# braingeneers/statdepth

Measured on AMD Instinct MI355X. Metric: curve-pairs/sec (MBD), higher is better.
Workload: dtype f64

## Files before the change

### statdepth_amd/csrc/mbd_rank_bucket32.hip

```cpp
#include <atomic>

#include "sd_common.h"
#include "rank_routes.h"
#include "rank_bucket.h"

namespace sd {

constexpr int R32_PRIO_LDS = 2;
constexpr int R32_PRIO_VALU = 0;
constexpr int R32_MIN_N = 3072;
constexpr int R32_LNB = 14;
constexpr int R32_NT = 512, R32_NW = 8;
constexpr int R32_LCAP = 64;
constexpr int R32_PAD = 12;
constexpr u32 R32_TB = 1024;
constexpr int R32_TSH = 30;
constexpr double R32_CDIV = 1.0 / 448.0;
constexpr double R32_BETA = 2.0;
constexpr u32 R32_SENT = 0x7FFFFFFFu;

template <int E, int LNB>
struct R32Cfg {
    static constexpr int NT = R32_NT, NW = R32_NW, NB = 1 << LNB;
    static constexpr int QW = NB / 2 / NT / 4;
    static_assert(QW >= 1 && NB / 2 == QW * 4 * NT, "whole quads of histogram words per thread");
    static constexpr int SH = 31 - LNB;
    static constexpr u32 C0 = R32_TB << SH, C1 = ((u32)NB - R32_TB) << SH;
    static constexpr u32 NANIMG = ((u32)NB + 2u) << SH;
    static_assert(LNB == 14, "the first tail octave continues the core's slope for 14 336 core buckets");
    static constexpr size_t HDR = 8 * NW * 8 + NW * 4 + 32 + (size_t)R32_LCAP * 8;
    static_assert(HDR % 16 == 0, "the histogram starts on a 16-byte boundary");
    static __host__ __device__ constexpr int al4(int n) { return (n + 3) & ~3; }
    static __host__ __device__ constexpr int pstride(int n) { return (n + 31) & ~31; }
    static __host__ __device__ constexpr int dummy_pos(int n) { return al4(n) + R32_PAD; }
    static __host__ __device__ constexpr size_t lds_bytes(int n) { return HDR + (size_t)(NB / 2 + 4) * 4 + (size_t)(dummy_pos(n) + 4) * 4; }
};

template <int E, int LNB>
__global__ __launch_bounds__(R32_NT, 4) void rank_bucket32_kernel(const double *__restrict__ Y, i64 n64, i64 row0, i64 rows,
                                                                 u32 *__restrict__ partial, unsigned char *__restrict__ rowflag,
                                                                 u32 *__restrict__ gate, u32 epoch, u64 *__restrict__ out_zero) {
    using C = R32Cfg<E, LNB>;
    constexpr int NT = C::NT, NW = C::NW, NB = C::NB, QW = C::QW, SH = C::SH;
    constexpr u32 C0 = C::C0, C1 = C::C1, NANIMG = C::NANIMG;
    extern __shared__ double Sm[];
    const int n = (int)n64;
    double *red = Sm;
    u32 *wtot = reinterpret_cast<u32 *>(red + 8 * NW);
    u32 *misc = wtot + NW;
    u32 *lkey = misc + 8, *lbe = lkey + R32_LCAP;
    u32 *H = reinterpret_cast<u32 *>(reinterpret_cast<char *>(Sm) + C::HDR);
    u32 *S = H + NB / 2 + 4;
    const unsigned short *H16 = reinterpret_cast<const unsigned short *>(H);
    const int t0 = threadIdx.x;
    const double INF = __builtin_huge_val();
    const double QNAN = __builtin_nan("");
    const int DUMMY = C::dummy_pos(n);
    const uint4 *SENT = reinterpret_cast<const uint4 *>(S + C::al4(n));
    const u32 nm1 = (u32)n - 1u;
    const u32 ranksum = (u32)(((u64)n * (u64)(n - 1)) >> 1);
    int t = t0;

    if (blockIdx.x == 0 && t == 0) gate[2] = 0;
    if (out_zero)
        for (i64 c = (i64)blockIdx.x * NT + t; c < n; c += (i64)gridDim.x * NT) out_zero[c] = 0;
    for (int p = n + t; p < DUMMY + 4; p += NT) S[p] = R32_SENT;
    {
        uint4 *Hq = reinterpret_cast<uint4 *>(H);
#pragma unroll
        for (int i = 0; i < QW; ++i) Hq[i * NT + t] = make_uint4(0, 0, 0, 0);
        if (t < 4) H[NB / 2 + t] = 0;
        if (t < 5) misc[t] = 0;
    }

    double x[E];
    auto load_row = [&](i64 r) {
        const double *rp = Y + (row0 + r) * n + t;
#pragma unroll
        for (int e = 0; e < E; ++e) x[e] = (e < E - 2 || t + e * NT < n) ? rp[e * NT] : QNAN;
    };
    u32 acc[E];
#pragma unroll
    for (int e = 0; e < E; ++e) acc[e] = 0;
    double smp;
    auto sample_issue = [&](i64 r) { smp = Y[(row0 + r) * n + (((((u32)t * 397u) & 511u) * (u32)n) >> 9)]; };
    auto row_range = [&](int parity) {
        double mn = INF, mx = -INF;
#pragma unroll
        for (int e = 0; e < E; ++e) {
            mn = rb_mm<false>(mn, x[e]);
            mx = rb_mm<true>(mx, x[e]);
        }
        mn = rb_wave_allreduce<false>(mn);
        mx = rb_wave_allreduce<true>(mx);
        const float sf = (float)smp;
        const float rmn = rb_row_allreduce_f32<false>(sf == sf ? sf : __builtin_huge_valf());
        const float rmx = rb_row_allreduce_f32<true>(sf == sf ? sf : -__builtin_huge_valf());
        auto rl = [](float v, int l) -> float { return __int_as_float(__builtin_amdgcn_readlane(__float_as_int(v), l)); };
        float imn = fmaxf(fmaxf(rl(rmn, 0), rl(rmn, 16)), fmaxf(rl(rmn, 32), rl(rmn, 48)));
        float imx = fminf(fminf(rl(rmx, 0), rl(rmx, 16)), fminf(rl(rmx, 32), rl(rmx, 48)));
        {
            bool eqs = false;
#define R32_NB(k) eqs = eqs || (__int_as_float(__builtin_amdgcn_mov_dpp(__float_as_int(sf), 0x120 + k, 0xF, 0xF, false)) == sf);
            R32_NB(1) R32_NB(2) R32_NB(3) R32_NB(4) R32_NB(5) R32_NB(6) R32_NB(7)
#undef R32_NB
            if (__ballot(eqs) != 0) { imn = __builtin_huge_valf(); imx = -__builtin_huge_valf(); }
        }
        double *rp = red + parity * 4 * NW;
        if ((t & 63) == 63) {
            double *wp = rp + 4 * (t >> 6);
            wp[0] = mn; wp[1] = mx;
            reinterpret_cast<float *>(wp + 2)[0] = imn;
            reinterpret_cast<float *>(wp + 2)[1] = imx;
        }
    };
    int par = 0;
    u32 rowidx = 0, nbad = 0, expect = 0;
    bool handover = false;
    bool stop = false;
    u32 kb[E];
    i64 r = blockIdx.x;
    for (; r < rows; r += gridDim.x) {
        t = t0;
        asm volatile("" : "+v"(t));
        const int lane = t & 63;
        const int wave = __builtin_amdgcn_readfirstlane(t >> 6);
        if (rowidx && t == 0) misc[3] = __hip_atomic_load(gate + 1, __ATOMIC_RELAXED, __HIP_MEMORY_SCOPE_AGENT);
        __builtin_amdgcn_s_setprio(R32_PRIO_LDS);
        sample_issue(r);
        load_row(r);
        row_range(par);
        double *redp = red + par * 4 * NW;
        par ^= 1;
        __syncthreads();
        if (rowidx) {
            const u32 w = misc[3];
            if ((w >> 8) == (epoch & 0xFFFFFFu) && (w & 0xFFu) >= 8u) { stop = true; break; }
        }
        double lo, hi;
        double mscale, moff, mc;
        u64 mcb;
        u32 mc0, mcw;
        bool go, bad;
        {
            const double2 p = reinterpret_cast<const double2 *>(redp)[2 * (lane & (NW - 1))];
            const float2 pb = reinterpret_cast<const float2 *>(redp + 4 * (lane & (NW - 1)) + 2)[0];
            lo = rb_readlane_f64(rb_row_allreduce<false>(p.x), 0);
            hi = rb_readlane_f64(rb_row_allreduce<true>(p.y), 0);
            const double imn = (double)__int_as_float(__builtin_amdgcn_readfirstlane(__float_as_int(rb_row_allreduce_f32<true>(pb.x))));
            const double imx = (double)__int_as_float(__builtin_amdgcn_readfirstlane(__float_as_int(rb_row_allreduce_f32<false>(pb.y))));
            const bool fin = (hi > lo) && (lo > -INF) && (hi < INF) && ((hi - lo) < INF);
            bad = !fin && (hi >= lo);
            const double si = imx - imn;
            u32 c0 = 256u, c1 = 0x7FFFFE00u;
            if (fin && si > 0.0 && si < INF && (hi - lo) > (1.5 * (1.0 + 2.0 * R32_BETA)) * si) {
                const double lo2 = imn - R32_BETA * si, hi2 = imx + R32_BETA * si;
                lo = lo2 > lo ? lo2 : lo;
                hi = hi2 < hi ? hi2 : hi;
                c0 = C0;
                c1 = C1;
            }
            mc0 = c0;
            mcw = c1 - c0;
            const double wc = hi - lo;
            mscale = ((double)mcw - 64.0) / wc;
            moff = __builtin_fma(-lo, mscale, (double)c0);
            mc = wc * R32_CDIV;
            mcb = (u64)__double_as_longlong(mc);
            go = fin && (wc > 0.0) && (mscale < INF) && (mc > 0.0);
            bad = bad || (fin && !go);
        }
        auto convert4 = [&](const double (&xv)[4], u32 (&q)[4], u32 (&bk)[4]) {
            bool anyout = false;
            u32 fr[4];
#pragma unroll
            for (int i = 0; i < 4; ++i) {
                const double u = __builtin_fma(xv[i], mscale, moff);
                u32 qi;
                asm("v_cvt_u32_f64 %0, %1" : "=v"(qi) : "v"(u));
                const double f = __builtin_amdgcn_fract(u) * 16384.0;
                asm("v_cvt_u32_f64 %0, %1" : "=v"(fr[i]) : "v"(f));
                q[i] = qi;
                anyout = anyout || (qi - mc0 >= mcw);
            }
            if (__ballot(anyout) != 0) {
#pragma unroll
                for (int i = 0; i < 4; ++i) {
                    const bool outc = q[i] - mc0 >= mcw, low = q[i] < mc0;
                    double d = low ? lo - xv[i] : xv[i] - hi;
                    d = rb_mm<true>(d, 0.0);
                    const u64 tc = ((u64)__double_as_longlong(d + mc) - mcb) >> R32_TSH;
                    const u32 room = low ? mc0 - 1u : 0x7FFFFEFFu - (mc0 + mcw);
                    const u32 tcc = tc < (u64)room ? (u32)tc : room;
                    u32 qt = low ? (mc0 - 1u) - tcc : (mc0 + mcw) + tcc;
                    qt = (xv[i] == xv[i]) ? qt : NANIMG;
                    q[i] = outc ? qt : q[i];
                    fr[i] = outc ? 0u : fr[i];
                }
            }
#pragma unroll
            for (int i = 0; i < 4; ++i) {
                bk[i] = q[i] >> SH;
                q[i] = ((q[i] << (31 - SH)) & 0x7FFFFFFFu) | fr[i];
            }
        };
        u32 bc[E];
        if (go) {

#pragma unroll
            for (int e0 = 0; e0 < E; e0 += 8) {
                u32 old[8];
#pragma unroll
                for (int h = 0; h < 8; h += 4) {
                    if (e0 + h < E) {
                        double xv[4];
                        u32 q[4], bk[4];
#pragma unroll
                        for (int i = 0; i < 4; ++i) xv[i] = e0 + h + i < E ? x[e0 + h + i] : x[e0 + h];
                        convert4(xv, q, bk);
#pragma unroll
                        for (int i = 0; i < 4; ++i)
                            if (e0 + h + i < E) { kb[e0 + h + i] = q[i]; bc[e0 + h + i] = bk[i]; }
                    }
                }
#pragma unroll
                for (int i = 0; i < 8; ++i) {
                    const int e = e0 + i;
                    if (e < E) {
                        const u32 b = bc[e];
                        old[i] = atomicAdd(&H[b >> 1], 1u << ((b & 1u) * 16u));
                    }
                }
#pragma unroll
                for (int i = 0; i < 8; ++i) {
                    const int e = e0 + i;
                    if (e < E)
                        bc[e] |= ((old[i] >> ((bc[e] & 1u) * 16u)) & 0xFFu) << 16;
                }
#pragma unroll
                for (int i = 0; i < 8; ++i)
                    if (e0 + i < E) asm volatile("" : "+v"(bc[e0 + i]));
            }
            __syncthreads();
            uint4 *Hq = reinterpret_cast<uint4 *>(H) + wave * (64 * QW);
            uint4 hq[QW];
            u32 runq[QW], inclq[QW], offq[QW], ov = 0, wsum = 0;
#pragma unroll
            for (int i = 0; i < QW; ++i) {
                hq[i] = Hq[i * 64 + lane];
                const u32 s4 = hq[i].x + hq[i].y + hq[i].z + hq[i].w;
                ov |= hq[i].x | hq[i].y | hq[i].z | hq[i].w;
                runq[i] = (s4 & 0xFFFFu) + (s4 >> 16);
                inclq[i] = rb_wave_incl_scan(runq[i]);
                offq[i] = wsum;
                wsum += rb_readlane(inclq[i], 63);
            }
            const bool wover = __ballot((ov & 0xFFC0FFC0u) != 0) != 0;
            const bool wtry = __ballot((ov & 0xFFF0FFF0u) != 0) != 0;
            if (lane == 63) wtot[wave] = wsum | (wover ? 0x80000000u : 0u) | (wtry ? 0x40000000u : 0u);
            __syncthreads();
            const u32 wt = wtot[lane & (NW - 1)];
            const bool crowded = __ballot((wt >> 31) != 0) != 0;
            const bool trypure = __ballot((wt & 0x40000000u) != 0) != 0;
            const u32 wscan = rb_row_incl_scan(wt & 0x3FFFFFFFu);
            const u32 woff = wave ? rb_readlane(wscan, wave - 1) : 0u;
#pragma unroll
            for (int i = 0; i < QW; ++i) {
                u32 base = woff + offq[i] + inclq[i] - runq[i];
                uint4 o;
                o.x = base | ((base + (hq[i].x & 0xFFFFu)) << 16);
                base += (hq[i].x & 0xFFFFu) + (hq[i].x >> 16);
                o.y = base | ((base + (hq[i].y & 0xFFFFu)) << 16);
                base += (hq[i].y & 0xFFFFu) + (hq[i].y >> 16);
                o.z = base | ((base + (hq[i].z & 0xFFFFu)) << 16);
                base += (hq[i].z & 0xFFFFu) + (hq[i].z >> 16);
                o.w = base | ((base + (hq[i].w & 0xFFFFu)) << 16);
                base += (hq[i].w & 0xFFFFu) + (hq[i].w >> 16);
                Hq[i * 64 + lane] = o;
                if (i == QW - 1 && t == NT - 1) H[NB / 2] = base;
            }
            __syncthreads();
            const u32 nv = H[NB / 2];
            bool take = nv == (u32)n;
            if (take) {
#pragma unroll
                for (int e = 0; e < E; ++e) {
                    const u32 b = bc[e] & 0xFFFFu, slot = bc[e] >> 16;
                    u32 b1 = b + 1u;
                    asm("" : "+v"(b1));
                    const u32 base = H16[b], end = H16[b1];
                    const bool isk = e < E - 2 || t + e * NT < n;
                    S[isk ? base + slot : (u32)DUMMY] = kb[e];
                    bc[e] = isk ? base | ((end - base) << 14) : (1u << 14);
                }
            }
            __syncthreads();
            bool pure = false;
            if (take && (trypure || crowded)) {
                const u32 tag = rowidx + 1u;
                bool vote = false, same = true;
#pragma unroll
                for (int e = 0; e < E; ++e) {
                    const u32 base = bc[e] & 0x3FFFu, cnt = bc[e] >> 14;
                    if (e < E - 2 || t + e * NT < n) {
                        const u32 first = S[base];
                        same = same && (first == kb[e]);
                        if (cnt >= 16u) vote = vote || (first == kb[e] && S[base + 1] == kb[e]);
                    }
                }
                if (vote) misc[2] = tag;
                if (!same) misc[4] = tag;
                __syncthreads();
                if ((misc[2] == tag && misc[4] != tag) || crowded) {
                    take = false;
                    bool ok = misc[2] == tag && misc[4] != tag;
                    if (ok) {
                        const double *rp = Y + (row0 + r) * n + t;
#pragma unroll
                        for (int pass = 0; pass < 2; ++pass) {
                            bool eq = true;
#pragma unroll
                            for (int e0 = 0; e0 < E; e0 += 4) {
                                int eo = e0 * NT;
                                asm volatile("" : "+v"(eo));
                                const double *rq = rp + eo;
                                u64 w[4];
#pragma unroll
                                for (int i = 0; i < 4; ++i) {
                                    const bool isk = e0 + i < E && (e0 + i < E - 2 || t + (e0 + i) * NT < n);
                                    w[i] = (u64)__double_as_longlong((isk ? rq[i * NT] : 0.0) + 0.0);
                                }
#pragma unroll
                                for (int i = 0; i < 4; ++i) {
                                    if (e0 + i < E && (e0 + i < E - 2 || t + (e0 + i) * NT < n) && (bc[e0 + i] >> 14) >= 2u) {
                                        u32 *sp = S + (bc[e0 + i] & 0x3FFFu);
                                        if (pass == 0) { sp[0] = (u32)(w[i] >> 32); sp[1] = (u32)w[i]; }
                                        else eq = eq && sp[0] == (u32)(w[i] >> 32) && sp[1] == (u32)w[i];
                                    }
                                }
                                __builtin_amdgcn_sched_barrier(0);
                            }
                            if (pass == 1 && !eq) misc[4] = tag;
                            __syncthreads();
                        }
                        ok = misc[4] != tag;
                    }
                    if (ok) {
                        pure = true;
#pragma unroll
                        for (int e = 0; e < E; ++e) {
                            const u32 B = bc[e] & 0x3FFFu, A = (u32)n - B - (bc[e] >> 14);
                            acc[e] += (e < E - 2 || t + e * NT < n) ? (nm1 * (nm1 - 1u) - A * (A - 1u) - B * (B - 1u)) >> 1 : 0u;
                        }
                    }
                }
            }
            __builtin_amdgcn_s_setprio(R32_PRIO_VALU);
            {
                uint4 *Hz = reinterpret_cast<uint4 *>(H) + wave * (64 * QW);
#pragma unroll
                for (int i = 0; i < QW; ++i) Hz[i * 64 + lane] = make_uint4(0, 0, 0, 0);
                if (t < 2) H[NB / 2 + t] = 0;
            }
            if (take) {
                const uint4 *S4 = reinterpret_cast<const uint4 *>(S);
                uint4 y0, y1;
                auto window = [&](int e) {
                    const u32 base = bc[e] & 0x3FFFu, cnt = bc[e] >> 14;
                    const uint4 *p = S4 + (base >> 2);
                    y0 = p[0];
                    y1 = *((cnt + (base & 3u) > 4u) ? p + 1 : SENT);
                };
                u32 sB = 0;
                window(0);
#pragma unroll
                for (int e = 0; e < E; ++e) {
                    const u32 base = bc[e] & 0x3FFFu, cnt = bc[e] >> 14, off = base & 3u;
                    const u32 qe = kb[e];
                    u32 lt = 0;
                    lt = __builtin_amdgcn_alignbit(lt, y1.w - qe, 31);
                    lt = __builtin_amdgcn_alignbit(lt, y1.z - qe, 31);
                    lt = __builtin_amdgcn_alignbit(lt, y1.y - qe, 31);
                    lt = __builtin_amdgcn_alignbit(lt, y1.x - qe, 31);
                    lt = __builtin_amdgcn_alignbit(lt, y0.w - qe, 31);
                    lt = __builtin_amdgcn_alignbit(lt, y0.z - qe, 31);
                    lt = __builtin_amdgcn_alignbit(lt, y0.y - qe, 31);
                    lt = __builtin_amdgcn_alignbit(lt, y0.x - qe, 31);
                    if (e + 1 < E) window(e + 1);
                    u32 less = (u32)__popc(__builtin_amdgcn_ubfe(lt, off, cnt < 8u ? cnt : 8u));
                    if (cnt + off > 8u) {
                        const uint4 *p = S4 + (base >> 2);
#pragma unroll 1
                        for (u32 kk = 8; kk < cnt + off; kk += 4) {
                            const uint4 y = p[kk >> 2];
                            const u32 rest = cnt + off - kk;
                            u32 l4 = 0;
                            l4 = __builtin_amdgcn_alignbit(l4, y.w - qe, 31);
                            l4 = __builtin_amdgcn_alignbit(l4, y.z - qe, 31);
                            l4 = __builtin_amdgcn_alignbit(l4, y.y - qe, 31);
                            l4 = __builtin_amdgcn_alignbit(l4, y.x - qe, 31);
                            less += (u32)__popc(__builtin_amdgcn_ubfe(l4, 0u, rest < 4u ? rest : 4u));
                        }
                    }
                    const u32 B = base + less;
                    kb[e] = B;
                    const bool isk = e < E - 2 || t + e * NT < n;
                    sB += isk ? B : 0u;
                    acc[e] += isk ? __umul24(B, nm1 - B) : 0u;
                    __builtin_amdgcn_sched_barrier(0);
                }
                sB = rb_wave_incl_scan(sB);
                if (lane == 63) atomicAdd(&misc[1], sB);
                __syncthreads();
                {
                    const u32 have_sum = misc[1];
                    expect += ranksum;
                    if (have_sum != expect) {
                        expect = have_sum;
                        const u32 l0 = misc[0];
#pragma unroll
                        for (int e = 0; e < E; ++e)
                            if (e < E - 2 || t + e * NT < n) atomicAdd(&H[kb[e] >> 1], 1u << ((kb[e] & 1u) * 16u));
                        __syncthreads();
#pragma unroll
                        for (int e = 0; e < E; ++e) {
                            if (e < E - 2 || t + e * NT < n) {
                                const u32 B = kb[e], c = H16[B];
                                if (c != 1u) {
                                    acc[e] -= __umul24(B, nm1 - B);
                                    const u32 idx = atomicAdd(&misc[0], 1u);
                                    if (idx < (u32)R32_LCAP) {
                                        lkey[idx] = (rowidx << 14) | (u32)(t + e * NT);
                                        lbe[idx] = B | (c << 16);
                                    }
                                }
                            }
                        }
                        __syncthreads();
                        if (E <= 16 && misc[0] > (u32)R32_LCAP) {
                            const u32 tag = (rowidx + 1u) | 0x40000000u;
                            const double *rp = Y + (row0 + r) * n + t;
#pragma unroll
                            for (int pass = 0; pass < 2; ++pass) {
                                bool eq = true;
#pragma unroll
                                for (int e0 = 0; e0 < E; e0 += 2) {
                                    int eo = e0 * NT;
                                    asm volatile("" : "+v"(eo));
                                    const double *rq = rp + eo;
                                    u64 w[2];
#pragma unroll
                                    for (int i = 0; i < 2; ++i) {
                                        const bool isk = e0 + i < E && (e0 + i < E - 2 || t + (e0 + i) * NT < n);
                                        w[i] = (u64)__double_as_longlong((isk ? rq[i * NT] : 0.0) + 0.0);
                                    }
#pragma unroll
                                    for (int i = 0; i < 2; ++i) {
                                        if (e0 + i < E && (e0 + i < E - 2 || t + (e0 + i) * NT < n) && H16[kb[e0 + i]] >= 2u) {
                                            u32 *sp = S + kb[e0 + i];
                                            if (pass == 0) { sp[0] = (u32)(w[i] >> 32); sp[1] = (u32)w[i]; }
                                            else eq = eq && sp[0] == (u32)(w[i] >> 32) && sp[1] == (u32)w[i];
                                        }
                                    }
                                    __builtin_amdgcn_sched_barrier(0);
                                }
                                if (pass == 1 && !eq) misc[4] = tag;
                                __syncthreads();
                            }
                            if (misc[4] != tag) {
#pragma unroll
                                for (int e = 0; e < E; ++e) {
                                    if (e < E - 2 || t + e * NT < n) {
                                        const u32 B = kb[e], c = H16[B];
                                        if (c != 1u) {
                                            const u32 A = (u32)n - B - c;
                                            acc[e] += (nm1 * (nm1 - 1u) - A * (A - 1u) - B * (B - 1u)) >> 1;
                                        }
                                    }
                                }
                                if (t == 0) misc[0] = l0;
                            }
                            __syncthreads();
                        }
#pragma unroll
                        for (int e = 0; e < E; ++e)
                            if (e < E - 2 || t + e * NT < n) H[kb[e] >> 1] = 0;
                        __syncthreads();
                        if (misc[0] > (u32)R32_LCAP) handover = true;
                    }
                }
            } else {
                bad = !pure;
            }
        }
        if (t == 0) rowflag[r] = bad ? 1 : 0;
        nbad += bad ? 1u : 0u;
        ++rowidx;
        if (handover) break;
        if (bad && rowidx == 1 && t == 0 && blockIdx.x < 16) {
            u32 old = gate[1], assumed;
            do {
                assumed = old;
                const u32 want = ((assumed >> 8) != (epoch & 0xFFFFFFu)) ? (((epoch & 0xFFFFFFu) << 8) | 1u)
                                 : ((assumed & 0xFFu) == 0xFFu ? assumed : assumed + 1u);
                old = atomicCAS(gate + 1, assumed, want);
            } while (old != assumed);
        }
        if (nbad >= 2 && 2 * nbad > rowidx) { stop = true; r += gridDim.x; break; }
    }
    t = t0;
    __syncthreads();
    const u32 L = __builtin_amdgcn_readfirstlane(handover ? 0u : misc[0]);
    if (handover) {
        for (i64 rr = blockIdx.x + (i64)t * gridDim.x; rr < rows; rr += (i64)NT * gridDim.x) rowflag[rr] = 1;
        nbad = 1;
#pragma unroll
        for (int e = 0; e < E; ++e) acc[e] = 0;
    } else if (stop) {
        for (i64 rr = r + (i64)t * gridDim.x; rr < rows; rr += (i64)NT * gridDim.x) rowflag[rr] = 1;
    }
    if (t == 0 && nbad) *gate = epoch;
    u32 key = 0, be = 0;
    double xv = 0.0;
    if ((u32)t < L) {
        key = lkey[t];
        be = lbe[t];
        xv = Y[(row0 + (i64)blockIdx.x + (i64)(key >> 14) * gridDim.x) * n + (key & 0x3FFFu)];
    }
    u32 *P = partial + (size_t)blockIdx.x * C::pstride(n);
#pragma unroll
    for (int e = 0; e < E; ++e)
        if (e < E - 2 || t + e * NT < n) __builtin_nontemporal_store(acc[e], &P[t + e * NT]);
    if (L) {
        asm volatile("s_waitcnt vmcnt(0)" ::: "memory");
        __syncthreads();
        if (t < 64) {
            u32 B = be & 0xFFFFu, A = (u32)n - B - (be >> 16);
            for (u32 j = 0; j < L; ++j) {
                const u32 kj = rb_readlane(key, (int)j), bj = rb_readlane(be, (int)j);
                const double xj = rb_readlane_f64(xv, (int)j);
                if (j != (u32)t && (kj >> 14) == (key >> 14) && (bj & 0xFFFFu) == (be & 0xFFFFu)) {
                    B += (xj < xv) ? 1u : 0u;
                    A += (xj > xv) ? 1u : 0u;
                }
            }
            if ((u32)t < L) atomicAdd(&P[key & 0x3FFFu], (nm1 * (nm1 - 1u) - A * (A - 1u) - B * (B - 1u)) >> 1);
        }
    }
}

bool rank_bucket32_supported(i64 n, i64 rows, int cus) {
    const u64 per = (u64)((rows + cus - 1) / cus) * (u64)n * (u64)n;
    return n > R32_MIN_N && n <= 11264 && rows >= cus && rows <= 4096 && per < ((u64)1 << 32) && xswitch("SD_RB_NO32") == 0;
}

size_t rank_bucket32_extra_bytes(i64 rows) { return align_up((size_t)rows + 64, 256); }

template <int E>
static int launch32_cfg(const double *Y, i64 n, i64 row0, i64 rows, u32 *partial, unsigned char *rowflag, u32 *gate, u32 epoch,
                        u64 *out_zero, int G, hipStream_t s) {
    using C = R32Cfg<E, R32_LNB>;
    auto kf = rank_bucket32_kernel<E, R32_LNB>;
    const size_t lds = C::lds_bytes((int)n);
    if (lds > 81920) return fail(SD_ERR_UNSUPPORTED, "bucket32 kernel: %zu bytes of LDS for n=%lld", lds, (long long)n);
    SD_HIP(hipFuncSetAttribute((const void *)kf, hipFuncAttributeMaxDynamicSharedMemorySize, (int)lds));
    hipLaunchKernelGGL(kf, dim3(G), dim3(R32_NT), lds, s, Y, n, row0, rows, partial, rowflag, gate, epoch, out_zero);
    SD_HIP(hipGetLastError());
    return SD_OK;
}

int launch_rank_bucket32(const double *Y, i64 n, i64 row0, i64 rows, u32 *partial, unsigned char *rowflag, u32 *gate, u32 epoch,
                         u64 *out_zero, int G, hipStream_t s) {
    switch ((int)((n + 1023) / 1024)) {
        case 3: return launch32_cfg<6>(Y, n, row0, rows, partial, rowflag, gate, epoch, out_zero, G, s);
        case 4: return launch32_cfg<8>(Y, n, row0, rows, partial, rowflag, gate, epoch, out_zero, G, s);
        case 5: return launch32_cfg<10>(Y, n, row0, rows, partial, rowflag, gate, epoch, out_zero, G, s);
        case 6: return launch32_cfg<12>(Y, n, row0, rows, partial, rowflag, gate, epoch, out_zero, G, s);
        case 7: return launch32_cfg<14>(Y, n, row0, rows, partial, rowflag, gate, epoch, out_zero, G, s);
        case 8: return launch32_cfg<16>(Y, n, row0, rows, partial, rowflag, gate, epoch, out_zero, G, s);
        case 9: return launch32_cfg<18>(Y, n, row0, rows, partial, rowflag, gate, epoch, out_zero, G, s);
        case 10: return launch32_cfg<20>(Y, n, row0, rows, partial, rowflag, gate, epoch, out_zero, G, s);
        case 11: return launch32_cfg<22>(Y, n, row0, rows, partial, rowflag, gate, epoch, out_zero, G, s);
    }
    return fail(SD_ERR_UNSUPPORTED, "bucket32 kernel covers 3072 < n <= 11264");
}

u32 rank_bucket32_epoch() {
    static std::atomic<u32> counter{0};
    u32 e = ++counter;
    if (e == 0) e = ++counter;
    return e;
}

}
```

Before: 2198 billion.

## Derive bucket keys from biased double bits and drop strided sample bracket

Per-element conversion no longer uses two f64-to-u32 conversions plus fract. It adds a 2^38 bias to the affine image and reads the bucket index and fraction directly from the double's bit pattern using alignbit and mask operations. The core bounds are also changed so they align with the high-word steps. The bracket estimate now comes from a per-wave helper over the loaded registers instead of a separate strided sample load plus row-wide float reductions. This removes one global load and several cross-wave reductions per row, at the cost of a different outlier bracket heuristic and tighter precision assumptions on the biased encoding.

```diff
diff --git a/statdepth_amd/csrc/mbd_rank_bucket32.hip b/statdepth_amd/csrc/mbd_rank_bucket32.hip
--- a/statdepth_amd/csrc/mbd_rank_bucket32.hip
+++ b/statdepth_amd/csrc/mbd_rank_bucket32.hip
@@ -17,6 +17,8 @@
 constexpr int R32_TSH = 30;
 constexpr double R32_CDIV = 1.0 / 448.0;
 constexpr double R32_BETA = 2.0;
+constexpr double R32_VBASE = 274877906944.0;
+constexpr u32 R32_VBASE_HI = 0x42500000u;
 constexpr u32 R32_SENT = 0x7FFFFFFFu;
 
 template <int E, int LNB>
@@ -26,6 +28,9 @@
     static_assert(QW >= 1 && NB / 2 == QW * 4 * NT, "whole quads of histogram words per thread");
     static constexpr int SH = 31 - LNB;
     static constexpr u32 C0 = R32_TB << SH, C1 = ((u32)NB - R32_TB) << SH;
+    static constexpr u32 CU0 = 2u << SH, CU1 = ((u32)NB - 2u) << SH;
+    static_assert(C0 % (2u << SH) == 0 && C1 % (2u << SH) == 0 && CU0 % (2u << SH) == 0 && CU1 % (2u << SH) == 0,
+                  "the core's bounds are whole steps of the high word of 2^38 + image (2^18 images)");
     static constexpr u32 NANIMG = ((u32)NB + 2u) << SH;
     static_assert(LNB == 14, "the first tail octave continues the core's slope for 14 336 core buckets");
     static constexpr size_t HDR = 8 * NW * 8 + NW * 4 + 32 + (size_t)R32_LCAP * 8;
@@ -42,7 +47,7 @@
                                                                  u32 *__restrict__ gate, u32 epoch, u64 *__restrict__ out_zero) {
     using C = R32Cfg<E, LNB>;
     constexpr int NT = C::NT, NW = C::NW, NB = C::NB, QW = C::QW, SH = C::SH;
-    constexpr u32 C0 = C::C0, C1 = C::C1, NANIMG = C::NANIMG;
+    constexpr u32 C0 = C::C0, C1 = C::C1, CU0 = C::CU0, CU1 = C::CU1, NANIMG = C::NANIMG;
     extern __shared__ double Sm[];
     const int n = (int)n64;
     double *red = Sm;
@@ -82,8 +87,6 @@
     u32 acc[E];
 #pragma unroll
     for (int e = 0; e < E; ++e) acc[e] = 0;
-    double smp;
-    auto sample_issue = [&](i64 r) { smp = Y[(row0 + r) * n + (((((u32)t * 397u) & 511u) * (u32)n) >> 9)]; };
     auto row_range = [&](int parity) {
         double mn = INF, mx = -INF;
 #pragma unroll
@@ -91,21 +94,16 @@
             mn = rb_mm<false>(mn, x[e]);
             mx = rb_mm<true>(mx, x[e]);
         }
+        float2 wb = rb3_wave_bracket<E, NT>(mn, mx);
+        {
+            bool eqs = false;
+#pragma unroll
+            for (int e = 0; e < (E - 1 < 10 ? E - 1 : 10); ++e) eqs = eqs || (x[e] == x[e + 1]);
+            if (__ballot(eqs) != 0) { wb.x = __builtin_huge_valf(); wb.y = -__builtin_huge_valf(); }
+        }
+        const float imn = wb.x, imx = wb.y;
         mn = rb_wave_allreduce<false>(mn);
         mx = rb_wave_allreduce<true>(mx);
-        const float sf = (float)smp;
-        const float rmn = rb_row_allreduce_f32<false>(sf == sf ? sf : __builtin_huge_valf());
-        const float rmx = rb_row_allreduce_f32<true>(sf == sf ? sf : -__builtin_huge_valf());
-        auto rl = [](float v, int l) -> float { return __int_as_float(__builtin_amdgcn_readlane(__float_as_int(v), l)); };
-        float imn = fmaxf(fmaxf(rl(rmn, 0), rl(rmn, 16)), fmaxf(rl(rmn, 32), rl(rmn, 48)));
-        float imx = fminf(fminf(rl(rmx, 0), rl(rmx, 16)), fminf(rl(rmx, 32), rl(rmx, 48)));
-        {
-            bool eqs = false;
-#define R32_NB(k) eqs = eqs || (__int_as_float(__builtin_amdgcn_mov_dpp(__float_as_int(sf), 0x120 + k, 0xF, 0xF, false)) == sf);
-            R32_NB(1) R32_NB(2) R32_NB(3) R32_NB(4) R32_NB(5) R32_NB(6) R32_NB(7)
-#undef R32_NB
-            if (__ballot(eqs) != 0) { imn = __builtin_huge_valf(); imx = -__builtin_huge_valf(); }
-        }
         double *rp = red + parity * 4 * NW;
         if ((t & 63) == 63) {
             double *wp = rp + 4 * (t >> 6);
@@ -127,7 +125,6 @@
         const int wave = __builtin_amdgcn_readfirstlane(t >> 6);
         if (rowidx && t == 0) misc[3] = __hip_atomic_load(gate + 1, __ATOMIC_RELAXED, __HIP_MEMORY_SCOPE_AGENT);
         __builtin_amdgcn_s_setprio(R32_PRIO_LDS);
-        sample_issue(r);
         load_row(r);
         row_range(par);
         double *redp = red + par * 4 * NW;
@@ -141,6 +138,7 @@
         double mscale, moff, mc;
         u64 mcb;
         u32 mc0, mcw;
+        u32 mh0, mhw;
         bool go, bad;
         {
             const double2 p = reinterpret_cast<const double2 *>(redp)[2 * (lane & (NW - 1))];
@@ -152,7 +150,7 @@
             const bool fin = (hi > lo) && (lo > -INF) && (hi < INF) && ((hi - lo) < INF);
             bad = !fin && (hi >= lo);
             const double si = imx - imn;
-            u32 c0 = 256u, c1 = 0x7FFFFE00u;
+            u32 c0 = CU0, c1 = CU1;
             if (fin && si > 0.0 && si < INF && (hi - lo) > (1.5 * (1.0 + 2.0 * R32_BETA)) * si) {
                 const double lo2 = imn - R32_BETA * si, hi2 = imx + R32_BETA * si;
                 lo = lo2 > lo ? lo2 : lo;
@@ -164,7 +162,9 @@
             mcw = c1 - c0;
             const double wc = hi - lo;
             mscale = ((double)mcw - 64.0) / wc;
-            moff = __builtin_fma(-lo, mscale, (double)c0);
+            moff = __builtin_fma(-lo, mscale, R32_VBASE + (double)c0);
+            mh0 = R32_VBASE_HI + (c0 >> (SH + 1));
+            mhw = mcw >> (SH + 1);
             mc = wc * R32_CDIV;
             mcb = (u64)__double_as_longlong(mc);
             go = fin && (wc > 0.0) && (mscale < INF) && (mc > 0.0);
@@ -172,21 +172,20 @@
         }
         auto convert4 = [&](const double (&xv)[4], u32 (&q)[4], u32 (&bk)[4]) {
             bool anyout = false;
-            u32 fr[4];
+            u32 vh[4];
 #pragma unroll
             for (int i = 0; i < 4; ++i) {
-                const double u = __builtin_fma(xv[i], mscale, moff);
-                u32 qi;
-                asm("v_cvt_u32_f64 %0, %1" : "=v"(qi) : "v"(u));
-                const double f = __builtin_amdgcn_fract(u) * 16384.0;
-                asm("v_cvt_u32_f64 %0, %1" : "=v"(fr[i]) : "v"(f));
-                q[i] = qi;
-                anyout = anyout || (qi - mc0 >= mcw);
+                const u64 w = (u64)__double_as_longlong(__builtin_fma(xv[i], mscale, moff));
+                vh[i] = (u32)(w >> 32);
+                q[i] = (u32)w;
+                anyout = anyout || (vh[i] - mh0 >= mhw);
             }
             if (__ballot(anyout) != 0) {
+                const double vlo = __longlong_as_double((long long)((u64)mh0 << 32));
 #pragma unroll
                 for (int i = 0; i < 4; ++i) {
-                    const bool outc = q[i] - mc0 >= mcw, low = q[i] < mc0;
+                    const bool outc = vh[i] - mh0 >= mhw;
+                    const bool low = __longlong_as_double((long long)(((u64)vh[i] << 32) | q[i])) < vlo;
                     double d = low ? lo - xv[i] : xv[i] - hi;
                     d = rb_mm<true>(d, 0.0);
                     const u64 tc = ((u64)__double_as_longlong(d + mc) - mcb) >> R32_TSH;
@@ -194,14 +193,14 @@
                     const u32 tcc = tc < (u64)room ? (u32)tc : room;
                     u32 qt = low ? (mc0 - 1u) - tcc : (mc0 + mcw) + tcc;
                     qt = (xv[i] == xv[i]) ? qt : NANIMG;
-                    q[i] = outc ? qt : q[i];
-                    fr[i] = outc ? 0u : fr[i];
+                    vh[i] = outc ? qt >> (SH + 1) : vh[i];
+                    q[i] = outc ? qt << (31 - SH) : q[i];
                 }
             }
 #pragma unroll
             for (int i = 0; i < 4; ++i) {
-                bk[i] = q[i] >> SH;
-                q[i] = ((q[i] << (31 - SH)) & 0x7FFFFFFFu) | fr[i];
+                bk[i] = __builtin_amdgcn_alignbit(vh[i], q[i], 31) & 0x7FFFu;
+                q[i] &= 0x7FFFFFFFu;
             }
         };
         u32 bc[E];
```

Result: faster. 2351 billion, median of 6 (+7.0%).
